# lasgroup/Model-based-policy-optimizers

Measured on AMD Instinct MI355X. Metric: model-rollout transitions/sec + SAC updates/sec, Pendulum 5-ens h=5, higher is better.
Workload: dtype f32

## Files before the change

model-based-policy-optimizers_amd/csrc/lean_blocks.hpp:

```cpp
#pragma once
#include "common.hpp"
#include "chain_run.hpp"

#define MFMA(a, b, c) __builtin_amdgcn_mfma_f32_16x16x4f32((a), (b), (c), 0, 0, 0)

constexpr int LH = 64;
constexpr int LDH = 68;
constexpr int LT = 16 * LDH;
constexpr int LDX = 8;
constexpr int HID = LH * LH + LH;

struct ImgF {
  float w[16];
  float b[4];
};
__device__ __forceinline__ void img_fwd_request(ImgF &I, const float *__restrict__ W, int c0, int lane) {
  const int i = lane & 15, g = lane >> 4;
  const float *p = W + (16 * g) * LH + c0 + i;
#pragma unroll
  for (int s = 0; s < 16; ++s) I.w[s] = p[s * LH];
  const f4u t = *reinterpret_cast<const f4u *>(W + LH * LH + c0 + 4 * g);
  I.b[0] = t[0]; I.b[1] = t[1]; I.b[2] = t[2]; I.b[3] = t[3];
}
template <int N>
// ... 79 lines not shown
    }
  }
  float zv[4];
#pragma unroll
  for (int i = 0; i < 4; ++i) zv[i] = acc[i] + I.b[i];
  const int o = j * LDH + c0 + 4 * g;
  if (STORE_Z) {
    float dv[4];
    swish_and_grad4(zv, dv);
    store_vec_lds<4>(z_out + o, dv);
  } else {
    act_apply_vec<4>(zv, MBPO_ACT_SWISH);
  }
  store_vec_lds<4>(h_out + o, zv);
}
__device__ __forceinline__ void hid_fwd_jvp(const ImgF &I, const float *xin, const float *tin, float *h_out, float *t_out, int c0, int lane) {
  const int j = lane & 15, g = lane >> 4;
  float av[16], tv_in[16];
  read_row16(av, xin, lane);
  read_row16(tv_in, tin, lane);
  f32x4 acc = {0.f, 0.f, 0.f, 0.f}, tacc = {0.f, 0.f, 0.f, 0.f};
#pragma unroll
  for (int s = 0; s < 16; ++s) {
    acc = MFMA(I.w[s], av[s], acc);
    tacc = MFMA(I.w[s], tv_in[s], tacc);
  }
  float zv[4], tv[4];
#pragma unroll
  for (int i = 0; i < 4; ++i) {
    zv[i] = acc[i] + I.b[i];
    tv[i] = tacc[i];
  }
#pragma unroll
  for (int i = 0; i < 4; ++i) {
    const float sg = fast_sigmoid(zv[i]);
    tv[i] *= sg * (1.0f + zv[i] * (1.0f - sg));
    zv[i] = zv[i] * sg;
  }
  const int o = j * LDH + c0 + 4 * g;
  store_vec_lds<4>(t_out + o, tv);
  store_vec_lds<4>(h_out + o, zv);
}
__device__ __forceinline__ f32x4 out_fwd(const float (&w)[16], const float *xin, int lane) {
  float av[16];
  read_row16(av, xin, lane);
  f32x4 acc = {0.f, 0.f, 0.f, 0.f};
#pragma unroll
  for (int s = 0; s < 16; ++s) acc = MFMA(w[s], av[s], acc);
  return acc;
}
__device__ __forceinline__ void out_fwd2(const float (&w)[16], const float *xin, const float *tin, int lane, f32x4 &y, f32x4 &ty) {
  float av[16], tv[16];
  read_row16(av, xin, lane);
  read_row16(tv, tin, lane);
  f32x4 acc = {0.f, 0.f, 0.f, 0.f}, tacc = {0.f, 0.f, 0.f, 0.f};
#pragma unroll
  for (int s = 0; s < 16; ++s) {
    acc = MFMA(w[s], av[s], acc);
    tacc = MFMA(w[s], tv[s], tacc);
  }
  y = acc;
  ty = tacc;
}
template <class ST = NoSt>
__device__ __forceinline__ void hid_dgrad(const float (&w)[16], const float *din, const float *zprev, float *d_out, int k0, int lane, ST st = ST()) {
  const int j = lane & 15, g = lane >> 4;
  float av[16];
  st(0);
  read_row16(av, din, lane);
  const int o = j * LDH + k0 + 4 * g;
  float zv[4];
  load_vec_lds<4>(zprev + o, zv);
  st(1);
  f32x4 acc = {0.f, 0.f, 0.f, 0.f};
#pragma unroll
  for (int n = 0; n < 16; ++n) acc = MFMA(w[n], av[n], acc);
  float ov[4];
  st(2);
#pragma unroll
  for (int i = 0; i < 4; ++i) ov[i] = acc[i] * zv[i];
  store_vec_lds<4>(d_out + o, ov);
  st(3);
}
template <class ST = NoSt>
__device__ __forceinline__ void hid_wgrad(const float *hin, const float *delta, float *gst, int c0, int lane, ST st = ST()) {
  const int r = lane & 15, g = lane >> 4;
  st(0);
  f32x4 acc[4], accb = {0.f, 0.f, 0.f, 0.f};
#pragma unroll
  for (int a = 0; a < 4; ++a) acc[a] = (f32x4){0.f, 0.f, 0.f, 0.f};
  float hv[4][4], dv[4];
#pragma unroll
  for (int s = 0; s < 4; ++s) {
    const int row = 4 * g + s;
    load_vec_lds<4>(hin + row * LDH + 4 * r, hv[s]);
    dv[s] = delta[row * LDH + c0 + r];
  }
  const float one0 = (r == 0) ? 1.f : 0.f;
  st(1);
#pragma unroll
  for (int s = 0; s < 4; ++s) {
#pragma unroll
    for (int a = 0; a < 4; ++a) acc[a] = MFMA(dv[s], hv[s][a], acc[a]);
    accb = MFMA(dv[s], one0, accb);
  }
  st(2);
#pragma unroll
  for (int a = 0; a < 4; ++a) {
    const float ov[4] = {acc[a][0], acc[a][1], acc[a][2], acc[a][3]};
    store_vec_lds<4>(gst + (4 * r + a) * LH + 4 * (((c0 >> 2) + g + r) & 15), ov);
  }
  if (r == 0) {
    const float ov[4] = {accb[0], accb[1], accb[2], accb[3]};
    store_vec_lds<4>(gst + LH * LH + c0 + 4 * g, ov);
  }
  st(3);
}

__device__ __forceinline__ void copy_stage_out(const float *gst, float *__restrict__ gW, int t, int n_part, int q_begin = 0, int q_end = 1040) {
  for (int q = q_begin + t; q < q_end; q += n_part) {
    float v[4];
    load_vec_lds<4>(gst + 4 * q, v);
    int dst = 4 * q;
    if (q < 1024) {
      const int k = q >> 4, cc = q & 15;
      dst = k * LH + 4 * ((cc - (k >> 2)) & 15);
    }
    store_vec_global<4>(gW + dst, v);
  }
}

template <int CTRL>
__device__ __forceinline__ float dpp_shl(float v) {
  return __int_as_float(__builtin_amdgcn_update_dpp(0, __float_as_int(v), CTRL, 0xF, 0xF, true));
}
__device__ __forceinline__ float row_sum16(float v) {
  v += dpp_shl<0x108>(v);
  v += dpp_shl<0x104>(v);
  v += dpp_shl<0x102>(v);
  v += dpp_shl<0x101>(v);
  return v;
}

template <int K, bool STORE_Z, bool TANGENT>
__device__ __forceinline__ void thin_first(const float (&tw)[K + 1], const float *x, float *h0, float *z0, float *t0, int sub, int lane) {
  float xv[4][8];
#pragma unroll
  for (int i = 0; i < 4; ++i) {
    load_vec_lds<4>(x + (4 * sub + i) * LDX, *reinterpret_cast<float(*)[4]>(&xv[i][0]));
    if (K > 4) load_vec_lds<4>(x + (4 * sub + i) * LDX + 4, *reinterpret_cast<float(*)[4]>(&xv[i][4]));
  }
  float zv[4];
#pragma unroll
  for (int i = 0; i < 4; ++i) {
    float z = tw[K];
#pragma unroll
    for (int k = 0; k < K; ++k) z = fmaf(xv[i][k], tw[k], z);
    zv[i] = z;
  }
  if (TANGENT) {
    float tv[4] = {tw[K - 1], tw[K - 1], tw[K - 1], tw[K - 1]};
    act_grad_mul_vec<4>(tv, zv, MBPO_ACT_SWISH);
#pragma unroll
    for (int i = 0; i < 4; ++i) t0[(4 * sub + i) * LDH + lane] = tv[i];
  }
  if (STORE_Z) {
    float dv[4];
    swish_and_grad4(zv, dv);
#pragma unroll
    for (int i = 0; i < 4; ++i) z0[(4 * sub + i) * LDH + lane] = dv[i];
  } else {
    act_apply_vec<4>(zv, MBPO_ACT_SWISH);
  }
#pragma unroll
  for (int i = 0; i < 4; ++i) h0[(4 * sub + i) * LDH + lane] = zv[i];
}
template <int N>
__device__ __forceinline__ void thin_dgrad_last(const float (&two)[N], const float *dY, const float (&zv)[4], float *d_out, int sub, int lane) {
  float dv[4][N], sv[4];
#pragma unroll
  for (int i = 0; i < 4; ++i)
#pragma unroll
    for (int o = 0; o < N; ++o) dv[i][o] = dY[(4 * sub + i) * 4 + o];
#pragma unroll
  for (int i = 0; i < 4; ++i) {
    float s = 0.f;
#pragma unroll
    for (int o = 0; o < N; ++o) s = fmaf(dv[i][o], two[o], s);
    sv[i] = s * zv[i];
  }
#pragma unroll
  for (int i = 0; i < 4; ++i) d_out[(4 * sub + i) * LDH + lane] = sv[i];
}
__device__ __forceinline__ void thin_z_preload(float (&zv)[4], const float *z2, int sub, int lane) {
#pragma unroll
  for (int i = 0; i < 4; ++i) zv[i] = z2[(4 * sub + i) * LDH + lane];
}
template <int N>
__device__ __forceinline__ void thin_wgrad_last(const float (&hc)[16], const float *dY, float *__restrict__ gW, int sub, int lane) {
  if (sub < N) {
    float dv[16];
#pragma unroll
    for (int r = 0; r < 16; ++r) dv[r] = dY[r * 4 + sub];
    float acc = 0.f;
#pragma unroll
    for (int r = 0; r < 16; ++r) acc = fmaf(hc[r], dv[r], acc);
    gW[lane * N + sub] = acc;
  }
  if (sub == 0 && lane < N) {
    float acc = 0.f;
#pragma unroll
    for (int r = 0; r < 16; ++r) acc += dY[r * 4 + lane];
    gW[LH * N + lane] = acc;
  }
}
__device__ __forceinline__ void thin_col_preload(float (&hc)[16], const float *h2, int lane) {
#pragma unroll
  for (int r = 0; r < 16; ++r) hc[r] = h2[r * LDH + lane];
}
template <int K>
__device__ __forceinline__ void thin_wgrad_first_(const float *x, const float *d0, float *__restrict__ gW, int w8, int lane) {
  if (w8 > K) return;
  float dv[16];
#pragma unroll
  for (int r = 0; r < 16; ++r) dv[r] = d0[r * LDH + lane];
  if (w8 < K) {
    float acc = 0.f;
#pragma unroll
    for (int r = 0; r < 16; ++r) acc = fmaf(x[r * LDX + w8], dv[r], acc);
    gW[w8 * LH + lane] = acc;
  } else {
    float acc = 0.f;
#pragma unroll
    for (int r = 0; r < 16; ++r) acc += dv[r];
    gW[K * LH + lane] = acc;
  }
}

struct Img0 {
  float w[2][2];
};

__device__ __forceinline__ void in_fwd2(const Img0 &I, const float *bias, const float *x, int kc, int K, float *h_out, int c0, int lane) {
  const int j = lane & 15, g = lane >> 4;
  float xs[2];
#pragma unroll
  for (int s = 0; s < 2; ++s) {
    const int k = g * kc + s;
    const bool ok = (s < kc) && (k < K);
    const float v = x[j * LDX + (ok ? k : 0)];
    xs[s] = ok ? v : 0.f;
  }
#pragma unroll
  for (int t = 0; t < 2; ++t) {
    f32x4 acc = {0.f, 0.f, 0.f, 0.f};
    acc = MFMA(I.w[t][0], xs[0], acc);
    acc = MFMA(I.w[t][1], xs[1], acc);
    float zv[4], bv[4];
    load_vec_lds<4>(bias + c0 + 16 * t + 4 * g, bv);
#pragma unroll
    for (int q = 0; q < 4; ++q) zv[q] = acc[q] + bv[q];
    act_apply_vec<4>(zv, MBPO_ACT_SWISH);
    store_vec_lds<4>(h_out + j * LDH + c0 + 16 * t + 4 * g, zv);
  }
}

__device__ __forceinline__ void hid_fwd2(const float (&wa)[16], const float (&wb)[16], const float *bias, const float *xin, float *h_out, int c0,
                                         int lane) {
  const int j = lane & 15, g = lane >> 4;
  float av[16];
  read_row16(av, xin, lane);
  f32x4 a = {0.f, 0.f, 0.f, 0.f}, b = {0.f, 0.f, 0.f, 0.f};
#pragma unroll
  for (int s = 0; s < 16; ++s) {
    a = MFMA(wa[s], av[s], a);
    b = MFMA(wb[s], av[s], b);
  }
  float za[4], zb[4], ba[4], bb[4];
  load_vec_lds<4>(bias + c0 + 4 * g, ba);
  load_vec_lds<4>(bias + c0 + 16 + 4 * g, bb);
#pragma unroll
  for (int q = 0; q < 4; ++q) {
    za[q] = a[q] + ba[q];
    zb[q] = b[q] + bb[q];
  }
  act_apply_vec<4>(za, MBPO_ACT_SWISH);
  act_apply_vec<4>(zb, MBPO_ACT_SWISH);
  store_vec_lds<4>(h_out + j * LDH + c0 + 4 * g, za);
  store_vec_lds<4>(h_out + j * LDH + c0 + 16 + 4 * g, zb);
}
__device__ __forceinline__ void img_w_request(float (&w)[16], const float *__restrict__ W, int c0, int lane) {
  const int i = lane & 15, g = lane >> 4;
  const float *p = W + (16 * g) * LH + c0 + i;
#pragma unroll
  for (int s = 0; s < 16; ++s) w[s] = p[s * LH];
}
```

model-based-policy-optimizers_amd/csrc/sac_lean.hip:

```cpp
#include "common.hpp"
#include "chain_run.hpp"
#include "lean_blocks.hpp"
#include "sac_shared.hpp"
#include "sac_lean.hpp"

namespace {

template <int X>
struct Net {
  static constexpr int KP = X, KQ = X + 1, D = 2 * X + 4;
  static constexpr int P_W1 = KP * LH + LH, P_OUT = P_W1 + 2 * HID, P = P_OUT + LH * 2 + 2;
  static constexpr int Q_W1 = KQ * LH + LH, Q_OUT = Q_W1 + 2 * HID, Q = Q_OUT + LH + 1;
};

constexpr int O_QIN = 0;
constexpr int O_QIN2 = 128;
constexpr int O_AUX = 256;
constexpr int O_EPS = 320;
constexpr int O_EPS2 = 336;
constexpr int O_LP = 352;
constexpr int O_A = 368, O_SIG = 384, O_RAW = 400;
constexpr int O_Q = 416;
constexpr int O_DQ = 448;
constexpr int O_QOLD = 480;
constexpr int O_DY = 496;
constexpr int O_FLAG = 560;
constexpr int O_TILES = 564;
constexpr int N_TILES = 14;
constexpr int N_AUX = 3;
constexpr int LEAN_THREADS = 64 * (8 + N_AUX);
constexpr int O_STAGE = O_TILES + N_TILES * LT;
constexpr int GST = LH * LH + LH;
constexpr size_t LEAN_LDS_BYTES = (size_t)(O_STAGE + 2 * GST) * sizeof(float);

#define LEAN_STAMP(i)                                                                   \
  if (STAMPS) {                                                                         \
    if (A.stamps && tile == 0 && tid == 0) {                                            \
      unsigned long long t_;                                                            \
      asm volatile("s_memtime %0\n\ts_waitcnt lgkmcnt(0)" : "=s"(t_)::"memory");        \
      A.stamps[(trole == 1 ? 16 : 0) + (i)] = t_;                                       \
    }                                                                                   \
  }

}

#define FINE_STAMP(w, i)                                                                \
  if (STAMPS) {                                                                         \
    if (A.stamps && tile == 0 && trole == 0 && wave == (w) && lane == 0) {              \
      unsigned long long t_;                                                            \
      asm volatile("s_memtime %0\n\ts_waitcnt lgkmcnt(0)" : "=s"(t_)::"memory");        \
      A.stamps[32 + (i)] = t_;                                                          \
    }                                                                                   \
  }

template <int X, bool STAMPS>
__global__ void __launch_bounds__(LEAN_THREADS) k_sac_lean(const SacLeanArgs A) {
  extern __shared__ __align__(16) float smem[];
  using N = Net<X>;
  constexpr int D = N::D, KP = N::KP, KQ = N::KQ;
  static_assert(X >= 1 && X + 1 <= LDX, "x + u must fit an 8-column input tile");
  const int tid_ = threadIdx.x;
  const int wave = __builtin_amdgcn_readfirstlane(tid_ >> 6);
  const int c = wave >> 2, sub = wave & 3, c0 = sub * 16;
  const int trole = blockIdx.x % 3, tile = blockIdx.x / 3;
  const float *a_params = A.params, *a_target_q = A.target_q, *a_batch = A.batch, *a_norm_mean = A.norm_mean, *a_norm_std = A.norm_std;
  float *a_slab_pi = A.slab_pi, *a_slab_q = A.slab_q;
  int B = A.B;
  asm volatile("" : "+s"(a_params), "+s"(a_target_q), "+s"(a_batch), "+s"(a_norm_mean), "+s"(a_norm_std), "+s"(a_slab_pi), "+s"(a_slab_q), "+s"(B));
  const int row0 = tile * 16;
  {
    const int tid = tid_;
    LEAN_STAMP(0);
  }
  const float invB = 1.0f / (float)B;

  float *const s_qin = smem + O_QIN, *const s_qin2 = smem + O_QIN2, *const s_aux = smem + O_AUX;
  float *const tiles = smem + O_TILES;
#define TILE(n) (tiles + (n) * LT)

  auto aux_clip_words = [&]() __attribute__((always_inline)) {
    const uint4 qw0 = *reinterpret_cast<const uint4 *>(A.opt.seq), qw1 = *reinterpret_cast<const uint4 *>(A.opt.seq + 4);
    const unsigned int seq_issued = qw0.x, seq_resolved = qw0.y;
    const bool odd = (seq_issued & 1u) == 0u;
    const float q0 = __uint_as_float(odd ? qw1.y : qw0.z), q1 = __uint_as_float(odd ? qw1.z : qw0.w), q2 = __uint_as_float(odd ? qw1.w : qw1.x);
    const float lim = (A.opt.max_norm / A.opt.grad_scale) * (A.opt.max_norm / A.opt.grad_scale) * 0.9998f;
    const bool maybe = seq_issued != seq_resolved && !(q0 < lim && q1 < lim && q2 < lim);
    if (tid_ == 512) smem[O_FLAG] = maybe ? 1.f : 0.f;
    if (blockIdx.x == 0 && tid_ == 512) {
      const float count_in = A.step_count_rw[0];
      const unsigned int slot = qw0.x & 1u;
      A.opt.slot_word[0] = slot;
      float *q = reinterpret_cast<float *>(A.opt.seq) + 2 + 3 * slot;
      q[0] = 0.f; q[1] = 0.f; q[2] = 0.f;
      A.step_count_rw[0] = count_in + 1.0f;
      if (A.p2p_epoch) {
        const unsigned int ep0_in = A.p2p_epoch[0], ep1_in = A.p2p_epoch[1];
        A.p2p_epoch[0] = ep0_in + 1u;
        A.p2p_epoch[1] = ep1_in + A.p2p_blocks;
      }
    }
  };

  auto run = [&](const bool second_pass) __attribute__((always_inline)) {
    const int tid = opaque(tid_), lane = tid & 63;
    const float *const pi_p = a_params;
    const bool has_elem = tid < 16 * D;
    const int r_t = tid / D, cc_t = tid - r_t * D;
    const bool is_obs = cc_t < X, is_obs2 = cc_t >= X + 3 && cc_t < 2 * X + 3;
    const int oc_t = is_obs ? cc_t : (is_obs2 ? cc_t - (X + 3) : 0);
    float v_t = 0.f, mu_t = 0.f, sd_t = 1.f;
    if (has_elem && (trole != 1 || is_obs)) {
      const int nvalid = (B - row0 < 16 ? B - row0 : 16) * D;
      if (tid < nvalid) v_t = a_batch[(long long)row0 * D + tid];
      if (a_norm_mean && (is_obs || is_obs2)) {
        mu_t = a_norm_mean[oc_t];
        sd_t = a_norm_std[oc_t];
      }
    }
    auto tile_to_lds = [&]() __attribute__((always_inline)) {
      if (has_elem) {
        float v = v_t;
        if (a_norm_mean && (is_obs || is_obs2)) v = (v - mu_t) / sd_t;
        int dst = -1;
        if (is_obs) dst = O_QIN + r_t * LDX + cc_t;
        else if (trole != 1) {
          if (is_obs2) dst = O_QIN2 + r_t * LDX + oc_t;
          else if (cc_t == X) dst = O_QIN + r_t * LDX + X;
          else if (cc_t == X + 1) dst = O_AUX + r_t * 4 + 0;
          else if (cc_t == X + 2) dst = O_AUX + r_t * 4 + 1;
          else dst = O_AUX + r_t * 4 + 2;
        }
        if (dst >= 0) smem[dst] = v;
      }
    };
    if (wave >= 8) {
      const int ax = wave - 8;
      const bool critic = trole != 1;
      const int kq = trole >> 1;
      const RngKey rk = rng_resolve(A.seed, A.offset, A.rng_dev);
      const bool second = lane >= 16;
      const int r = lane & 15;
      const bool draws = ax == 0 && lane < (critic ? 16 : 32);
      const float *const given = critic ? A.noise_critic : (second ? A.noise_alpha : A.noise_actor);
      const unsigned int stream = critic ? MBPO_STREAM_SAC_CRITIC : (second ? MBPO_STREAM_SAC_ALPHA : MBPO_STREAM_SAC_ACTOR);
      const long long nidx = row0 + r;
      float e_given = 0.f;
      if (draws && given && row0 + r < B) e_given = given[nidx];
      __syncthreads();
      if (ax == 0 && !second_pass) aux_clip_words();
      __syncthreads();
      Philox4 bits;
      bits.v[0] = bits.v[1] = bits.v[2] = bits.v[3] = 0u;
      if (draws && !given) bits = philox_normal_bits(rk.seed, rk.offset, stream, (unsigned long long)nidx);
      __syncthreads();
      if (draws) {
        float e = 0.f;
        if (row0 + r < B) e = given ? e_given : philox_normal_from_bits(bits);
        smem[(second ? O_EPS2 : O_EPS) + r] = e;
      }
      __syncthreads();
      __syncthreads();
      __syncthreads();
      __syncthreads();
      const float log_alpha_v = second_pass ? __hip_atomic_load(a_params + N::P + 2 * N::Q, __ATOMIC_RELAXED, __HIP_MEMORY_SCOPE_AGENT)
                                            : a_params[N::P + 2 * N::Q];
      const float alpha = expf(log_alpha_v);
      const bool ok = row0 + r < B;
      if (critic) {
        float nlp = 0.f;
        nlp += smem[O_LP + r];
        const float rew = s_aux[r * 4 + 0], disc = s_aux[r * 4 + 1], trunc = s_aux[r * 4 + 2], qold = smem[O_QOLD + r];
        float gamma = A.discounting;
        if (A.neq) {
          const float pseudo = s_qin[r * LDX + X];
          float tfa = (A.neq_tu - A.neq_tl) / 2.0f * pseudo + (A.neq_tu + A.neq_tl) / 2.0f;
          tfa = floor_divide_f(tfa, A.neq_dt) * A.neq_dt;
          gamma = expf(-A.neq_cd * tfa);
        }
        __syncthreads();
        __syncthreads();
        float e2 = 0.f;
        if (ax == 0 && lane < 16) {
          const float nq = fminf(smem[O_Q + r], smem[O_Q + 16 + r]);
          const float next_v = nq - alpha * nlp;
          const float target = rew * A.reward_scaling + disc * gamma * next_v;
          const float err = ok ? (qold - target) * (1.f - trunc) : 0.f;
          e2 = err * err;
          smem[O_DY + r * 4] = err * (1.f - trunc) * (0.5f * invB);
        }
        const float acc = row_sum16(e2);
        if (ax == 0 && lane == 0) A.slab_ex[tile * 4 + (kq == 1 ? 3 : 0)] = acc;
      } else {
        float lp_al = 0.f, lp_ac = 0.f;
        lp_al += smem[O_EPS2 + r];
        lp_ac += smem[O_LP + r];
        const float a = smem[O_A + r], sg = smem[O_SIG + r], eps = smem[O_EPS + r], raw = smem[O_RAW + r];
        __syncthreads();
        __syncthreads();
        float l_al = 0.f, l_ac = 0.f;
        if (ax == 0 && lane < 16) {
          l_al = ok ? alpha * (-lp_al - A.target_entropy) : 0.f;
          const float q0 = smem[O_Q + r], q1 = smem[O_Q + 16 + r];
          const float mq = fminf(q0, q1);
          l_ac = ok ? (alpha * lp_ac - mq) : 0.f;
          float g0 = 0.f, g1 = 0.f;
          if (ok) {
            if (q0 < q1) g0 = -invB;
            else if (q1 < q0) g1 = -invB;
            else g0 = g1 = -0.5f * invB;
          }
          const float dLda = g0 * smem[O_DQ + r] + g1 * smem[O_DQ + 16 + r];
          const float gz = dLda * (1.f - a * a) + alpha * invB * 2.f * a;
          const float gsig = gz * eps - alpha * invB / sg;
          smem[O_DY + r * 4] = ok ? gz : 0.f;
          smem[O_DY + r * 4 + 1] = ok ? gsig * fast_sigmoid(raw) : 0.f;
        }
        const float al = row_sum16(l_al), ac = row_sum16(l_ac);
        if (ax == 0 && lane == 0) {
          A.slab_ex[tile * 4 + 1] = ac;
          A.slab_ex[tile * 4 + 2] = al;
        }
      }
      __syncthreads();
      __syncthreads();
      __syncthreads();
      float *const aslab = critic ? a_slab_q + (long long)tile * (2 * N::Q) + kq * N::Q : a_slab_pi + (long long)tile * N::P;
      const int w1 = critic ? N::Q_W1 : N::P_W1, kk = critic ? KQ : KP;
      FINE_STAMP(8, 16);
      copy_stage_out(smem + O_STAGE, aslab + w1 + HID, ax * 64 + lane, N_AUX * 64);
      FINE_STAMP(8, 17);
      __syncthreads();
      FINE_STAMP(8, 18);
      copy_stage_out(smem + O_STAGE + GST, aslab + w1, (7 - kk + ax) * 64 + lane, (7 - kk + N_AUX) * 64);
      FINE_STAMP(8, 19);
    } else if (trole != 1) {
      const int kq = trole >> 1;
      const float *const qk_p = a_params + N::P + kq * N::Q;
      const float *const qt_p = a_target_q + c * N::Q;
      float tw[KQ + 1];
      ImgF I1, I2;
      float wo[16];
      float bo0 = 0.f, bo1 = 0.f;
      if (c == 0) {
        thin_col_request<KP>(*reinterpret_cast<float(*)[KP + 1]>(&tw[0]), pi_p, lane);
        img_fwd_request(I1, pi_p + N::P_W1, c0, lane);
        if (sub == 0) {
          img_out_request<2>(wo, pi_p + N::P_OUT, lane);
          bo0 = pi_p[N::P_OUT + LH * 2];
          bo1 = pi_p[N::P_OUT + LH * 2 + 1];
        }
      } else {
        thin_col_request<KQ>(tw, qk_p, lane);
        img_fwd_request(I1, qk_p + N::Q_W1, c0, lane);
        if (sub == 1) {
          img_out_request<1>(wo, qk_p + N::Q_OUT, lane);
          bo0 = qk_p[N::Q_OUT + LH];
        }
      }
      tile_to_lds();
      __syncthreads();
      LEAN_STAMP(1);
      float tw1[KQ + 1];
      ImgF J1, J2;
      if (c == 0) thin_first<KP, false, false>(*reinterpret_cast<float(*)[KP + 1]>(&tw[0]), s_qin2, TILE(0), nullptr, nullptr, sub, lane);
      else thin_first<KQ, true, false>(tw, s_qin, TILE(7), TILE(4), nullptr, sub, lane);
      thin_col_request<KQ>(tw1, qt_p, lane);
      img_fwd_request(I2, (c == 0 ? pi_p + N::P_W1 : qk_p + N::Q_W1) + HID, c0, lane);
      __syncthreads();
      LEAN_STAMP(2);
      {
        auto pf = make_pf([&](int s) __attribute__((always_inline)) { img_fwd_request_piece(J1, qt_p + N::Q_W1, c0, lane, s); });
        if (c == 0) hid_fwd<false>(I1, TILE(0), TILE(1), nullptr, c0, lane, pf);
        else hid_fwd<true>(I1, TILE(7), TILE(8), TILE(5), c0, lane, pf);
      }
      __syncthreads();
      LEAN_STAMP(3);
      {
        auto pf = make_pf([&](int s) __attribute__((always_inline)) { img_fwd_request_piece(J2, qt_p + N::Q_W1 + HID, c0, lane, s); });
        if (c == 0) hid_fwd<false>(I2, TILE(1), TILE(0), nullptr, c0, lane, pf);
        else hid_fwd<true>(I2, TILE(8), TILE(9), TILE(6), c0, lane, pf);
      }
      __syncthreads();
      LEAN_STAMP(4);
      float wo1[16];
      float bt = 0.f;
      float two[1];
      float G2[16], G1[16];
      if (c == 0 && sub == 0) {
        const f32x4 y = out_fwd(wo, TILE(0), lane);
        const float loc = y[0] + bo0, raw = y[1] + bo1;
        const int j = lane & 15;
        const ActSample sm = normal_tanh_sample(loc, raw, smem[O_EPS + j]);
        if (lane < 16) {
          s_qin2[j * LDX + X] = sm.a;
          smem[O_LP + j] = sm.lp;
        }
      } else if (c == 1 && sub == 1) {
        const f32x4 y = out_fwd(wo, TILE(9), lane);
        if (lane < 16) smem[O_QOLD + lane] = y[0] + bo0;
      }
      if (sub == c + 1) {
        img_out_request<1>(wo1, qt_p + N::Q_OUT, lane);
        bt = qt_p[N::Q_OUT + LH];
      }
      if (c == 0) {
        two[0] = qk_p[N::Q_OUT + lane];
        img_dgrad_request(G2, qk_p + N::Q_W1 + HID, c0, lane);
        img_dgrad_request(G1, qk_p + N::Q_W1, c0, lane);
      }
      __syncthreads();
      LEAN_STAMP(5);
      thin_first<KQ, false, false>(tw1, s_qin2, TILE(2 * c), nullptr, nullptr, sub, lane);
      __syncthreads();
      LEAN_STAMP(6);
      hid_fwd<false>(J1, TILE(2 * c), TILE(2 * c + 1), nullptr, c0, lane);
      __syncthreads();
      LEAN_STAMP(7);
      hid_fwd<false>(J2, TILE(2 * c + 1), TILE(2 * c), nullptr, c0, lane);
      __syncthreads();
      LEAN_STAMP(8);
      float zq[4], hc[16];
      if (sub == c + 1) {
        const f32x4 y = out_fwd(wo1, TILE(2 * c), lane);
        if (lane < 16) smem[O_Q + 16 * c + lane] = y[0] + bt;
      }
      if (c == 0) thin_z_preload(zq, TILE(6), sub, lane);
      else if (sub == 0) thin_col_preload(hc, TILE(9), lane);
      __syncthreads();
      LEAN_STAMP(9);
      __syncthreads();
      LEAN_STAMP(10);
      float *const slab = a_slab_q + (long long)tile * (2 * N::Q) + kq * N::Q;
      if (c == 0) thin_dgrad_last<1>(two, smem + O_DY, zq, TILE(0), sub, lane);
      else if (sub == 0) thin_wgrad_last<1>(hc, smem + O_DY, slab + N::Q_OUT, sub, lane);
      __syncthreads();
      LEAN_STAMP(11);
      {
        auto st0 = [&](int i) __attribute__((always_inline)) { FINE_STAMP(0, i); };
        auto st4 = [&](int i) __attribute__((always_inline)) { FINE_STAMP(4, 8 + i); };
        if (c == 0) hid_dgrad(G2, TILE(0), TILE(5), TILE(1), c0, lane, st0);
        else hid_wgrad(TILE(8), TILE(0), smem + O_STAGE, c0, lane, st4);
      }
      FINE_STAMP(0, 4);
      FINE_STAMP(4, 12);
      __syncthreads();
      FINE_STAMP(0, 5);
      FINE_STAMP(4, 13);
      LEAN_STAMP(12);
      if (c == 0) hid_dgrad(G1, TILE(1), TILE(4), TILE(2), c0, lane);
      else hid_wgrad(TILE(7), TILE(1), smem + O_STAGE + GST, c0, lane);
      FINE_STAMP(0, 20);
      FINE_STAMP(4, 21);
      __syncthreads();
      FINE_STAMP(0, 22);
      LEAN_STAMP(13);
      if (wave <= KQ) thin_wgrad_first_<KQ>(s_qin, TILE(2), slab, wave, lane);
      else copy_stage_out(smem + O_STAGE + GST, slab + N::Q_W1, (wave - (KQ + 1)) * 64 + lane, (7 - KQ + N_AUX) * 64);
      LEAN_STAMP(14);
    } else {
      const float *const q_p = a_params + N::P + c * N::Q;
      float tw[KP + 1];
      ImgF I1, I2;
      float wo[16];
      float bo0 = 0.f, bo1 = 0.f;
      float tw1[KQ + 1];
      ImgF J1, J2;
      float wo1[16];
      float bq = 0.f;
      if (c == 0) {
        thin_col_request<KP>(tw, pi_p, lane);
        img_fwd_request(I1, pi_p + N::P_W1, c0, lane);
        if (sub == 0) {
          img_out_request<2>(wo, pi_p + N::P_OUT, lane);
          bo0 = pi_p[N::P_OUT + LH * 2];
          bo1 = pi_p[N::P_OUT + LH * 2 + 1];
        }
      }
      tile_to_lds();
      __syncthreads();
      LEAN_STAMP(1);
      if (c == 0) {
        thin_first<KP, true, false>(tw, s_qin, TILE(7), TILE(4), nullptr, sub, lane);
        thin_col_request<KQ>(tw1, q_p, lane);
        img_fwd_request(I2, pi_p + N::P_W1 + HID, c0, lane);
      } else {
        thin_col_request<KQ>(tw1, q_p, lane);
        img_fwd_request(J1, q_p + N::Q_W1, c0, lane);
        img_fwd_request(J2, q_p + N::Q_W1 + HID, c0, lane);
        if (sub == 2) {
          img_out_request<1>(wo1, q_p + N::Q_OUT, lane);
          bq = q_p[N::Q_OUT + LH];
        }
      }
      __syncthreads();
      LEAN_STAMP(2);
      if (c == 0) {
        auto pf = make_pf([&](int s) __attribute__((always_inline)) { img_fwd_request_piece(J1, q_p + N::Q_W1, c0, lane, s); });
        hid_fwd<true>(I1, TILE(7), TILE(8), TILE(5), c0, lane, pf);
      }
      __syncthreads();
      LEAN_STAMP(3);
      if (c == 0) {
        auto pf = make_pf([&](int s) __attribute__((always_inline)) { img_fwd_request_piece(J2, q_p + N::Q_W1 + HID, c0, lane, s); });
        hid_fwd<true>(I2, TILE(8), TILE(9), TILE(6), c0, lane, pf);
      }
      __syncthreads();
      LEAN_STAMP(4);
      float two[2];
      float G2[16], G1[16];
      if (wave == 0) {
        const f32x4 y = out_fwd(wo, TILE(9), lane);
        const float loc = y[0] + bo0, raw = y[1] + bo1;
        const int j = lane & 15, g = lane >> 4;
        const ActSample sm = normal_tanh_sample(loc, raw, smem[(g == 1 ? O_EPS2 : O_EPS) + j]);
        if (g == 0) {
          smem[O_LP + j] = sm.lp;
          smem[O_A + j] = sm.a;
          smem[O_SIG + j] = sm.sigma;
          smem[O_RAW + j] = raw;
          s_qin[j * LDX + X] = sm.a;
        } else if (g == 1) {
          smem[O_EPS2 + j] = sm.lp;
        }
      } else if (wave == 1) {
        img_out_request<1>(wo1, q_p + N::Q_OUT, lane);
        bq = q_p[N::Q_OUT + LH];
      }
      if (c == 0) {
        two[0] = pi_p[N::P_OUT + lane * 2];
        two[1] = pi_p[N::P_OUT + lane * 2 + 1];
        img_dgrad_request(G2, pi_p + N::P_W1 + HID, c0, lane);
        img_dgrad_request(G1, pi_p + N::P_W1, c0, lane);
      }
      __syncthreads();
      LEAN_STAMP(5);
      const int tv0 = c == 0 ? 0 : 10, tt0 = c == 0 ? 2 : 12;
      thin_first<KQ, false, true>(tw1, s_qin, TILE(tv0), nullptr, TILE(tt0), sub, lane);
      __syncthreads();
      LEAN_STAMP(6);
      hid_fwd_jvp(J1, TILE(tv0), TILE(tt0), TILE(tv0 + 1), TILE(tt0 + 1), c0, lane);
      __syncthreads();
      LEAN_STAMP(7);
      hid_fwd_jvp(J2, TILE(tv0 + 1), TILE(tt0 + 1), TILE(tv0), TILE(tt0), c0, lane);
      __syncthreads();
      LEAN_STAMP(8);
      float zq[4], hc[16];
      if (sub == c + 1) {
        f32x4 y, ty;
        out_fwd2(wo1, TILE(tv0), TILE(tt0), lane, y, ty);
        if (lane < 16) {
          smem[O_Q + 16 * c + lane] = y[0] + bq;
          smem[O_DQ + 16 * c + lane] = ty[0];
        }
      }
      if (c == 0) thin_z_preload(zq, TILE(6), sub, lane);
      else if (sub < 2 && sub != 2) thin_col_preload(hc, TILE(9), lane);
      __syncthreads();
      LEAN_STAMP(9);
      __syncthreads();
      LEAN_STAMP(10);
      float *const slab = a_slab_pi + (long long)tile * N::P;
      if (c == 0) thin_dgrad_last<2>(two, smem + O_DY, zq, TILE(0), sub, lane);
      else if (sub < 2) thin_wgrad_last<2>(hc, smem + O_DY, slab + N::P_OUT, sub, lane);
      __syncthreads();
      LEAN_STAMP(11);
      if (c == 0) hid_dgrad(G2, TILE(0), TILE(5), TILE(1), c0, lane);
      else hid_wgrad(TILE(8), TILE(0), smem + O_STAGE, c0, lane);
      __syncthreads();
      LEAN_STAMP(12);
      if (c == 0) hid_dgrad(G1, TILE(1), TILE(4), TILE(2), c0, lane);
      else hid_wgrad(TILE(7), TILE(1), smem + O_STAGE + GST, c0, lane);
      __syncthreads();
      LEAN_STAMP(13);
      if (wave <= KP) thin_wgrad_first_<KP>(s_qin, TILE(2), slab, wave, lane);
      else copy_stage_out(smem + O_STAGE + GST, slab + N::P_W1, (wave - (KP + 1)) * 64 + lane, (7 - KP + N_AUX) * 64);
      LEAN_STAMP(14);
    }
  };

  run(false);
  if (smem[O_FLAG] == 0.f) return;
  float *const s_gn = smem + O_DQ;
  __syncthreads();
  sac_group_norms(A.opt, s_gn, tid_);
  __syncthreads();
  if (s_gn[0] < A.opt.max_norm && s_gn[1] < A.opt.max_norm && s_gn[2] < A.opt.max_norm) return;
  if (blockIdx.x == 0 && tid_ == 0) A.opt.seq[SAC_CTL_CLIP_EVENTS] += 1u;
  sac_clip_fixup(A.opt, s_gn, opaque(tid_), LEAN_THREADS);
  __threadfence();
  __builtin_amdgcn_s_dcache_inv();
  __syncthreads();
  run(true);
}

namespace {

template <int X>
int launch_x(const SacLeanArgs &A, int n_tiles, hipStream_t st) {
  return mbpo_with_bool(A.stamps != nullptr, [&](auto STAMP) {
    return mbpo_launch<k_sac_lean<X, STAMP.value>>(3 * n_tiles, LEAN_THREADS, LEAN_LDS_BYTES, st, "sac_lean", A);
  });
}

}

bool sac_lean_supports(int x_dim, int u_dim, const int *policy_dims, int policy_layers, int policy_act, const int *q_dims, int q_layers, int q_act) {
  if (u_dim != 1 || x_dim < 2 || x_dim > 6) return false;
  if (policy_layers != 4 || q_layers != 4 || policy_act != MBPO_ACT_SWISH || q_act != MBPO_ACT_SWISH) return false;
  for (int l = 1; l <= 3; ++l)
    if (policy_dims[l] != LH || q_dims[l] != LH) return false;
  return policy_dims[0] == x_dim && policy_dims[4] == 2 && q_dims[0] == x_dim + 1 && q_dims[4] == 1;
}

int sac_lean_launch(const SacLeanArgs &A, int x_dim, int n_tiles, void *stream) {
  hipStream_t st = (hipStream_t)stream;
  if (x_dim == 3) return launch_x<3>(A, n_tiles, st);
  if (x_dim == 4) return launch_x<4>(A, n_tiles, st);
  if (x_dim == 2) return mbpo_launch<k_sac_lean<2, false>>(3 * n_tiles, LEAN_THREADS, LEAN_LDS_BYTES, st, "sac_lean", A);
  if (x_dim == 5) return mbpo_launch<k_sac_lean<5, false>>(3 * n_tiles, LEAN_THREADS, LEAN_LDS_BYTES, st, "sac_lean", A);
  if (x_dim == 6) return mbpo_launch<k_sac_lean<6, false>>(3 * n_tiles, LEAN_THREADS, LEAN_LDS_BYTES, st, "sac_lean", A);
  mbpo_set_error("sac_lean: x_dim %d has no instantiation", x_dim);
  return MBPO_ERR_UNSUPPORTED;
}
```

Baseline: 19.41 million.

## Fuse loss and output-layer backward into hidden-layer gradient stage in SAC kernel

Every main wave now recomputes the per-row critic and actor loss gradients redundantly. The output-layer delta is folded directly into the first hidden dgrad and wgrad, and the output-layer weights are staged in LDS. This removes the O_DY round-trip through shared memory, the separate thin dgrad and wgrad passes, and several block-wide barriers. Aux waves compute the output-layer weight gradient from the loss in registers via readlane. The cost is duplicated loss arithmetic, more register pressure, and extra shuffles and LDS reads of output weights.

```diff
diff --git a/model-based-policy-optimizers_amd/csrc/lean_blocks.hpp b/model-based-policy-optimizers_amd/csrc/lean_blocks.hpp
--- a/model-based-policy-optimizers_amd/csrc/lean_blocks.hpp
+++ b/model-based-policy-optimizers_amd/csrc/lean_blocks.hpp
@@ -185,39 +185,108 @@
   store_vec_lds<4>(d_out + o, ov);
   st(3);
 }
+template <class DV, class ST = NoSt>
+__device__ __forceinline__ void hid_wgrad_from(const float *hin, DV dvf, float *gst, int c0, int lane, ST st = ST()) {
+  const int r = lane & 15, g = lane >> 4;
+  st(0);
+  f32x4 acc[4], accb = {0.f, 0.f, 0.f, 0.f};
+#pragma unroll
+  for (int a = 0; a < 4; ++a) acc[a] = (f32x4){0.f, 0.f, 0.f, 0.f};
+  float hv[4][4], dv[4];
+#pragma unroll
+  for (int s = 0; s < 4; ++s) {
+    load_vec_lds<4>(hin + (4 * g + s) * LDH + 4 * r, hv[s]);
+    dv[s] = dvf(s);
+  }
+  const float one0 = (r == 0) ? 1.f : 0.f;
+  st(1);
+#pragma unroll
+  for (int s = 0; s < 4; ++s) {
+#pragma unroll
+    for (int a = 0; a < 4; ++a) acc[a] = MFMA(dv[s], hv[s][a], acc[a]);
+    accb = MFMA(dv[s], one0, accb);
+  }
+  st(2);
+#pragma unroll
+  for (int a = 0; a < 4; ++a) {
+    const float ov[4] = {acc[a][0], acc[a][1], acc[a][2], acc[a][3]};
+    store_vec_lds<4>(gst + (4 * r + a) * LH + 4 * (((c0 >> 2) + g + r) & 15), ov);
+  }
+  if (r == 0) {
+    const float ov[4] = {accb[0], accb[1], accb[2], accb[3]};
+    store_vec_lds<4>(gst + LH * LH + c0 + 4 * g, ov);
+  }
+  st(3);
+}
 template <class ST = NoSt>
 __device__ __forceinline__ void hid_wgrad(const float *hin, const float *delta, float *gst, int c0, int lane, ST st = ST()) {
   const int r = lane & 15, g = lane >> 4;
+  hid_wgrad_from(hin, [&](int s) __attribute__((always_inline)) { return delta[(4 * g + s) * LDH + c0 + r]; }, gst, c0, lane, st);
+}
+
+template <int N>
+__device__ __forceinline__ float delta_last(const float (&dy)[N], const float (&wrow)[N], float zd) {
+  float s = 0.f;
+#pragma unroll
+  for (int o = 0; o < N; ++o) s = fmaf(dy[o], wrow[o], s);
+  return s * zd;
+}
+template <int N>
+__device__ __forceinline__ void lds_wout_rows(float (&w)[16][N], const float *wout, int lane) {
+  const float *p = wout + 16 * N * (lane >> 4);
+  float *const f = &w[0][0];
+#pragma unroll
+  for (int q = 0; q < 4 * N; ++q) load_vec_lds<4>(p + 4 * q, *reinterpret_cast<float(*)[4]>(&f[4 * q]));
+}
+template <int N>
+__device__ __forceinline__ void rows_of_group(float (&dy4)[4][N], const float (&dy)[N], int lane) {
+  const int g = lane >> 4;
+#pragma unroll
+  for (int s = 0; s < 4; ++s)
+#pragma unroll
+    for (int o = 0; o < N; ++o) dy4[s][o] = __shfl(dy[o], 4 * g + s, 64);
+}
+template <int N, class ST = NoSt>
+__device__ __forceinline__ void hid_dgrad_out(const float (&w)[16], const float (&dy)[N], const float (&wout)[16][N], float (&zd2)[16], const float *zprev,
+                                              float *d_out, int k0, int lane, ST st = ST()) {
+  const int j = lane & 15, g = lane >> 4;
   st(0);
-  f32x4 acc[4], accb = {0.f, 0.f, 0.f, 0.f};
-#pragma unroll
-  for (int a = 0; a < 4; ++a) acc[a] = (f32x4){0.f, 0.f, 0.f, 0.f};
-  float hv[4][4], dv[4];
-#pragma unroll
-  for (int s = 0; s < 4; ++s) {
-    const int row = 4 * g + s;
-    load_vec_lds<4>(hin + row * LDH + 4 * r, hv[s]);
-    dv[s] = delta[row * LDH + c0 + r];
-  }
-  const float one0 = (r == 0) ? 1.f : 0.f;
+  const int o = j * LDH + k0 + 4 * g;
+  float zv[4];
+  load_vec_lds<4>(zprev + o, zv);
+#pragma unroll
+  for (int n = 0; n < 16; ++n) zd2[n] = delta_last<N>(dy, wout[n], zd2[n]);
   st(1);
-#pragma unroll
-  for (int s = 0; s < 4; ++s) {
-#pragma unroll
-    for (int a = 0; a < 4; ++a) acc[a] = MFMA(dv[s], hv[s][a], acc[a]);
-    accb = MFMA(dv[s], one0, accb);
-  }
+  f32x4 acc = {0.f, 0.f, 0.f, 0.f};
+#pragma unroll
+  for (int n = 0; n < 16; ++n) acc = MFMA(w[n], zd2[n], acc);
+  float ov[4];
   st(2);
 #pragma unroll
-  for (int a = 0; a < 4; ++a) {
-    const float ov[4] = {acc[a][0], acc[a][1], acc[a][2], acc[a][3]};
-    store_vec_lds<4>(gst + (4 * r + a) * LH + 4 * (((c0 >> 2) + g + r) & 15), ov);
-  }
-  if (r == 0) {
-    const float ov[4] = {accb[0], accb[1], accb[2], accb[3]};
-    store_vec_lds<4>(gst + LH * LH + c0 + 4 * g, ov);
-  }
+  for (int i = 0; i < 4; ++i) ov[i] = acc[i] * zv[i];
+  store_vec_lds<4>(d_out + o, ov);
   st(3);
+}
+template <int N, class ST = NoSt>
+__device__ __forceinline__ void hid_wgrad_out(const float *hin, const float (&dy)[4][N], const float (&wcol)[N], const float (&zd)[4], float *gst, int c0,
+                                              int lane, ST st = ST()) {
+  hid_wgrad_from(hin, [&](int s) __attribute__((always_inline)) { return delta_last<N>(dy[s], wcol, zd[s]); }, gst, c0, lane, st);
+}
+template <int N>
+__device__ __forceinline__ void out_wgrad_col(const float (&hc)[16], float dy, float *__restrict__ gW, int o, int lane) {
+  float dv[16];
+#pragma unroll
+  for (int r = 0; r < 16; ++r) dv[r] = __int_as_float(__builtin_amdgcn_readlane(__float_as_int(dy), r));
+  float acc = 0.f;
+#pragma unroll
+  for (int r = 0; r < 16; ++r) acc = fmaf(hc[r], dv[r], acc);
+  gW[lane * N + o] = acc;
+  if (lane == 0) {
+    float b = 0.f;
+#pragma unroll
+    for (int r = 0; r < 16; ++r) b += dv[r];
+    gW[LH * N + o] = b;
+  }
 }
 
 __device__ __forceinline__ void copy_stage_out(const float *gst, float *__restrict__ gW, int t, int n_part, int q_begin = 0, int q_end = 1040) {
@@ -299,24 +368,6 @@
 #pragma unroll
   for (int i = 0; i < 4; ++i) zv[i] = z2[(4 * sub + i) * LDH + lane];
 }
-template <int N>
-__device__ __forceinline__ void thin_wgrad_last(const float (&hc)[16], const float *dY, float *__restrict__ gW, int sub, int lane) {
-  if (sub < N) {
-    float dv[16];
-#pragma unroll
-    for (int r = 0; r < 16; ++r) dv[r] = dY[r * 4 + sub];
-    float acc = 0.f;
-#pragma unroll
-    for (int r = 0; r < 16; ++r) acc = fmaf(hc[r], dv[r], acc);
-    gW[lane * N + sub] = acc;
-  }
-  if (sub == 0 && lane < N) {
-    float acc = 0.f;
-#pragma unroll
-    for (int r = 0; r < 16; ++r) acc += dY[r * 4 + lane];
-    gW[LH * N + lane] = acc;
-  }
-}
 __device__ __forceinline__ void thin_col_preload(float (&hc)[16], const float *h2, int lane) {
 #pragma unroll
   for (int r = 0; r < 16; ++r) hc[r] = h2[r * LDH + lane];
diff --git a/model-based-policy-optimizers_amd/csrc/sac_lean.hip b/model-based-policy-optimizers_amd/csrc/sac_lean.hip
--- a/model-based-policy-optimizers_amd/csrc/sac_lean.hip
+++ b/model-based-policy-optimizers_amd/csrc/sac_lean.hip
@@ -23,9 +23,9 @@
 constexpr int O_Q = 416;
 constexpr int O_DQ = 448;
 constexpr int O_QOLD = 480;
-constexpr int O_DY = 496;
 constexpr int O_FLAG = 560;
-constexpr int O_TILES = 564;
+constexpr int O_WOUT = 564;
+constexpr int O_TILES = O_WOUT + 128;
 constexpr int N_TILES = 14;
 constexpr int N_AUX = 3;
 constexpr int LEAN_THREADS = 64 * (8 + N_AUX);
@@ -41,6 +41,78 @@
       A.stamps[(trole == 1 ? 16 : 0) + (i)] = t_;                                       \
     }                                                                                   \
   }
+
+struct LossArgs {
+  int neq;
+  float discounting, reward_scaling, target_entropy, neq_cd, neq_tl, neq_tu, neq_dt;
+};
+struct CriticRow {
+  float nlp, rew, disc, trunc, qold, gamma;
+};
+struct CriticLoss {
+  float dy, e2;
+};
+template <int X>
+__device__ __forceinline__ CriticRow critic_row_preload(const float *smem, const LossArgs &A, int r) {
+  CriticRow p;
+  float nlp = 0.f;
+  nlp += smem[O_LP + r];
+  p.nlp = nlp;
+  p.rew = smem[O_AUX + r * 4 + 0], p.disc = smem[O_AUX + r * 4 + 1], p.trunc = smem[O_AUX + r * 4 + 2], p.qold = smem[O_QOLD + r];
+  float gamma = A.discounting;
+  if (A.neq) {
+    const float pseudo = smem[O_QIN + r * LDX + X];
+    float tfa = (A.neq_tu - A.neq_tl) / 2.0f * pseudo + (A.neq_tu + A.neq_tl) / 2.0f;
+    tfa = floor_divide_f(tfa, A.neq_dt) * A.neq_dt;
+    gamma = expf(-A.neq_cd * tfa);
+  }
+  p.gamma = gamma;
+  return p;
+}
+__device__ __forceinline__ CriticLoss critic_loss_row(const float *smem, const CriticRow &p, float alpha, float reward_scaling, bool ok, float invB, int r) {
+  const float nq = fminf(smem[O_Q + r], smem[O_Q + 16 + r]);
+  const float next_v = nq - alpha * p.nlp;
+  const float target = p.rew * reward_scaling + p.disc * p.gamma * next_v;
+  const float err = ok ? (p.qold - target) * (1.f - p.trunc) : 0.f;
+  CriticLoss l;
+  l.e2 = err * err;
+  l.dy = err * (1.f - p.trunc) * (0.5f * invB);
+  return l;
+}
+struct ActorRow {
+  float lp_al, lp_ac, a, sg, eps, raw;
+};
+struct ActorLoss {
+  float dy[2], l_al, l_ac;
+};
+__device__ __forceinline__ ActorRow actor_row_preload(const float *smem, int r) {
+  ActorRow p;
+  float lp_al = 0.f, lp_ac = 0.f;
+  lp_al += smem[O_EPS2 + r];
+  lp_ac += smem[O_LP + r];
+  p.lp_al = lp_al, p.lp_ac = lp_ac;
+  p.a = smem[O_A + r], p.sg = smem[O_SIG + r], p.eps = smem[O_EPS + r], p.raw = smem[O_RAW + r];
+  return p;
+}
+__device__ __forceinline__ ActorLoss actor_loss_row(const float *smem, const ActorRow &p, float alpha, float target_entropy, bool ok, float invB, int r) {
+  ActorLoss l;
+  l.l_al = ok ? alpha * (-p.lp_al - target_entropy) : 0.f;
+  const float q0 = smem[O_Q + r], q1 = smem[O_Q + 16 + r];
+  const float mq = fminf(q0, q1);
+  l.l_ac = ok ? (alpha * p.lp_ac - mq) : 0.f;
+  float g0 = 0.f, g1 = 0.f;
+  if (ok) {
+    if (q0 < q1) g0 = -invB;
+    else if (q1 < q0) g1 = -invB;
+    else g0 = g1 = -0.5f * invB;
+  }
+  const float dLda = g0 * smem[O_DQ + r] + g1 * smem[O_DQ + 16 + r];
+  const float gz = dLda * (1.f - p.a * p.a) + alpha * invB * 2.f * p.a;
+  const float gsig = gz * p.eps - alpha * invB / p.sg;
+  l.dy[0] = ok ? gz : 0.f;
+  l.dy[1] = ok ? gsig * fast_sigmoid(p.raw) : 0.f;
+  return l;
+}
 
 }
 
@@ -67,6 +139,9 @@
   float *a_slab_pi = A.slab_pi, *a_slab_q = A.slab_q;
   int B = A.B;
   asm volatile("" : "+s"(a_params), "+s"(a_target_q), "+s"(a_batch), "+s"(a_norm_mean), "+s"(a_norm_std), "+s"(a_slab_pi), "+s"(a_slab_q), "+s"(B));
+  LossArgs LA = {A.neq, A.discounting, A.reward_scaling, A.target_entropy, A.neq_cd, A.neq_tl, A.neq_tu, A.neq_dt};
+  asm volatile("" : "+s"(LA.neq), "+s"(LA.discounting), "+s"(LA.reward_scaling), "+s"(LA.target_entropy), "+s"(LA.neq_cd), "+s"(LA.neq_tl), "+s"(LA.neq_tu),
+               "+s"(LA.neq_dt));
   const int row0 = tile * 16;
   {
     const int tid = tid_;
@@ -74,7 +149,7 @@
   }
   const float invB = 1.0f / (float)B;
 
-  float *const s_qin = smem + O_QIN, *const s_qin2 = smem + O_QIN2, *const s_aux = smem + O_AUX;
+  float *const s_qin = smem + O_QIN, *const s_qin2 = smem + O_QIN2;
   float *const tiles = smem + O_TILES;
 #define TILE(n) (tiles + (n) * LT)
 
@@ -133,6 +208,9 @@
         if (dst >= 0) smem[dst] = v;
       }
     };
+    auto load_log_alpha = [&]() __attribute__((always_inline)) {
+      return second_pass ? __hip_atomic_load(a_params + N::P + 2 * N::Q, __ATOMIC_RELAXED, __HIP_MEMORY_SCOPE_AGENT) : a_params[N::P + 2 * N::Q];
+    };
     if (wave >= 8) {
       const int ax = wave - 8;
       const bool critic = trole != 1;
@@ -148,6 +226,12 @@
       if (draws && given && row0 + r < B) e_given = given[nidx];
       __syncthreads();
       if (ax == 0 && !second_pass) aux_clip_words();
+      const float *const wout_p = critic ? a_params + N::P + kq * N::Q + N::Q_OUT : a_params + N::P_OUT;
+      float wout0 = 0.f, wout1 = 0.f;
+      if (ax == 1) {
+        wout0 = wout_p[lane];
+        if (!critic) wout1 = wout_p[64 + lane];
+      }
       __syncthreads();
       Philox4 bits;
       bits.v[0] = bits.v[1] = bits.v[2] = bits.v[3] = 0u;
@@ -158,73 +242,46 @@
         if (row0 + r < B) e = given ? e_given : philox_normal_from_bits(bits);
         smem[(second ? O_EPS2 : O_EPS) + r] = e;
       }
-      __syncthreads();
-      __syncthreads();
-      __syncthreads();
-      __syncthreads();
-      const float log_alpha_v = second_pass ? __hip_atomic_load(a_params + N::P + 2 * N::Q, __ATOMIC_RELAXED, __HIP_MEMORY_SCOPE_AGENT)
-                                            : a_params[N::P + 2 * N::Q];
-      const float alpha = expf(log_alpha_v);
+      if (ax == 1) {
+        smem[O_WOUT + lane] = wout0;
+        if (!critic) smem[O_WOUT + 64 + lane] = wout1;
+      }
+      __syncthreads();
+      __syncthreads();
+      __syncthreads();
+      __syncthreads();
+      const float alpha = expf(load_log_alpha());
       const bool ok = row0 + r < B;
+      float *const aslab = critic ? a_slab_q + (long long)tile * (2 * N::Q) + kq * N::Q : a_slab_pi + (long long)tile * N::P;
+      float hc[16];
+      if (ax >= 1) thin_col_preload(hc, TILE(9), lane);
       if (critic) {
-        float nlp = 0.f;
-        nlp += smem[O_LP + r];
-        const float rew = s_aux[r * 4 + 0], disc = s_aux[r * 4 + 1], trunc = s_aux[r * 4 + 2], qold = smem[O_QOLD + r];
-        float gamma = A.discounting;
-        if (A.neq) {
-          const float pseudo = s_qin[r * LDX + X];
-          float tfa = (A.neq_tu - A.neq_tl) / 2.0f * pseudo + (A.neq_tu + A.neq_tl) / 2.0f;
-          tfa = floor_divide_f(tfa, A.neq_dt) * A.neq_dt;
-          gamma = expf(-A.neq_cd * tfa);
-        }
+        const CriticRow pr = critic_row_preload<X>(smem, LA, r);
         __syncthreads();
         __syncthreads();
-        float e2 = 0.f;
-        if (ax == 0 && lane < 16) {
-          const float nq = fminf(smem[O_Q + r], smem[O_Q + 16 + r]);
-          const float next_v = nq - alpha * nlp;
-          const float target = rew * A.reward_scaling + disc * gamma * next_v;
-          const float err = ok ? (qold - target) * (1.f - trunc) : 0.f;
-          e2 = err * err;
-          smem[O_DY + r * 4] = err * (1.f - trunc) * (0.5f * invB);
-        }
-        const float acc = row_sum16(e2);
-        if (ax == 0 && lane == 0) A.slab_ex[tile * 4 + (kq == 1 ? 3 : 0)] = acc;
+        const CriticLoss l = critic_loss_row(smem, pr, alpha, LA.reward_scaling, ok, invB, r);
+        if (ax == 0) {
+          const float acc = row_sum16(lane < 16 ? l.e2 : 0.f);
+          if (lane == 0) A.slab_ex[tile * 4 + (kq == 1 ? 3 : 0)] = acc;
+        } else if (ax == 1) {
+          out_wgrad_col<1>(hc, l.dy, aslab + N::Q_OUT, 0, lane);
+        }
       } else {
-        float lp_al = 0.f, lp_ac = 0.f;
-        lp_al += smem[O_EPS2 + r];
-        lp_ac += smem[O_LP + r];
-        const float a = smem[O_A + r], sg = smem[O_SIG + r], eps = smem[O_EPS + r], raw = smem[O_RAW + r];
+        const ActorRow pr = actor_row_preload(smem, r);
         __syncthreads();
         __syncthreads();
-        float l_al = 0.f, l_ac = 0.f;
-        if (ax == 0 && lane < 16) {
-          l_al = ok ? alpha * (-lp_al - A.target_entropy) : 0.f;
-          const float q0 = smem[O_Q + r], q1 = smem[O_Q + 16 + r];
-          const float mq = fminf(q0, q1);
-          l_ac = ok ? (alpha * lp_ac - mq) : 0.f;
-          float g0 = 0.f, g1 = 0.f;
-          if (ok) {
-            if (q0 < q1) g0 = -invB;
-            else if (q1 < q0) g1 = -invB;
-            else g0 = g1 = -0.5f * invB;
+        const ActorLoss l = actor_loss_row(smem, pr, alpha, LA.target_entropy, ok, invB, r);
+        if (ax == 0) {
+          const float al = row_sum16(lane < 16 ? l.l_al : 0.f), ac = row_sum16(lane < 16 ? l.l_ac : 0.f);
+          if (lane == 0) {
+            A.slab_ex[tile * 4 + 1] = ac;
+            A.slab_ex[tile * 4 + 2] = al;
           }
-          const float dLda = g0 * smem[O_DQ + r] + g1 * smem[O_DQ + 16 + r];
-          const float gz = dLda * (1.f - a * a) + alpha * invB * 2.f * a;
-          const float gsig = gz * eps - alpha * invB / sg;
-          smem[O_DY + r * 4] = ok ? gz : 0.f;
-          smem[O_DY + r * 4 + 1] = ok ? gsig * fast_sigmoid(raw) : 0.f;
-        }
-        const float al = row_sum16(l_al), ac = row_sum16(l_ac);
-        if (ax == 0 && lane == 0) {
-          A.slab_ex[tile * 4 + 1] = ac;
-          A.slab_ex[tile * 4 + 2] = al;
-        }
-      }
-      __syncthreads();
-      __syncthreads();
-      __syncthreads();
-      float *const aslab = critic ? a_slab_q + (long long)tile * (2 * N::Q) + kq * N::Q : a_slab_pi + (long long)tile * N::P;
+        } else {
+          out_wgrad_col<2>(hc, ax == 1 ? l.dy[0] : l.dy[1], aslab + N::P_OUT, ax - 1, lane);
+        }
+      }
+      __syncthreads();
       const int w1 = critic ? N::Q_W1 : N::P_W1, kk = critic ? KQ : KP;
       FINE_STAMP(8, 16);
       copy_stage_out(smem + O_STAGE, aslab + w1 + HID, ax * 64 + lane, N_AUX * 64);
@@ -284,7 +341,6 @@
       LEAN_STAMP(4);
       float wo1[16];
       float bt = 0.f;
-      float two[1];
       float G2[16], G1[16];
       if (c == 0 && sub == 0) {
         const f32x4 y = out_fwd(wo, TILE(0), lane);
@@ -304,10 +360,10 @@
         bt = qt_p[N::Q_OUT + LH];
       }
       if (c == 0) {
-        two[0] = qk_p[N::Q_OUT + lane];
         img_dgrad_request(G2, qk_p + N::Q_W1 + HID, c0, lane);
         img_dgrad_request(G1, qk_p + N::Q_W1, c0, lane);
       }
+      const float log_alpha_v = load_log_alpha();
       __syncthreads();
       LEAN_STAMP(5);
       thin_first<KQ, false, false>(tw1, s_qin2, TILE(2 * c), nullptr, nullptr, sub, lane);
@@ -319,44 +375,53 @@
       hid_fwd<false>(J2, TILE(2 * c + 1), TILE(2 * c), nullptr, c0, lane);
       __syncthreads();
       LEAN_STAMP(8);
-      float zq[4], hc[16];
+      const int lj = lane & 15, lg = lane >> 4;
       if (sub == c + 1) {
         const f32x4 y = out_fwd(wo1, TILE(2 * c), lane);
         if (lane < 16) smem[O_Q + 16 * c + lane] = y[0] + bt;
       }
-      if (c == 0) thin_z_preload(zq, TILE(6), sub, lane);
-      else if (sub == 0) thin_col_preload(hc, TILE(9), lane);
+      const float alpha = expf(log_alpha_v);
+      const CriticRow pr = critic_row_preload<X>(smem, LA, lj);
+      float wrow[16][1], wcol[1], zd2[16], zdw[4];
+      if (c == 0) {
+        read_row16(zd2, TILE(6), lane);
+        lds_wout_rows<1>(wrow, smem + O_WOUT, lane);
+      } else {
+        wcol[0] = smem[O_WOUT + c0 + lj];
+#pragma unroll
+        for (int s = 0; s < 4; ++s) zdw[s] = TILE(6)[(4 * lg + s) * LDH + c0 + lj];
+      }
       __syncthreads();
       LEAN_STAMP(9);
-      __syncthreads();
-      LEAN_STAMP(10);
       float *const slab = a_slab_q + (long long)tile * (2 * N::Q) + kq * N::Q;
-      if (c == 0) thin_dgrad_last<1>(two, smem + O_DY, zq, TILE(0), sub, lane);
-      else if (sub == 0) thin_wgrad_last<1>(hc, smem + O_DY, slab + N::Q_OUT, sub, lane);
-      __syncthreads();
-      LEAN_STAMP(11);
       {
         auto st0 = [&](int i) __attribute__((always_inline)) { FINE_STAMP(0, i); };
         auto st4 = [&](int i) __attribute__((always_inline)) { FINE_STAMP(4, 8 + i); };
-        if (c == 0) hid_dgrad(G2, TILE(0), TILE(5), TILE(1), c0, lane, st0);
-        else hid_wgrad(TILE(8), TILE(0), smem + O_STAGE, c0, lane, st4);
+        const float dy[1] = {critic_loss_row(smem, pr, alpha, LA.reward_scaling, row0 + lj < B, invB, lj).dy};
+        if (c == 0) {
+          hid_dgrad_out<1>(G2, dy, wrow, zd2, TILE(5), TILE(1), c0, lane, st0);
+        } else {
+          float dy4[4][1];
+          rows_of_group<1>(dy4, dy, lane);
+          hid_wgrad_out<1>(TILE(8), dy4, wcol, zdw, smem + O_STAGE, c0, lane, st4);
+        }
       }
       FINE_STAMP(0, 4);
       FINE_STAMP(4, 12);
       __syncthreads();
       FINE_STAMP(0, 5);
       FINE_STAMP(4, 13);
-      LEAN_STAMP(12);
+      LEAN_STAMP(10);
       if (c == 0) hid_dgrad(G1, TILE(1), TILE(4), TILE(2), c0, lane);
       else hid_wgrad(TILE(7), TILE(1), smem + O_STAGE + GST, c0, lane);
       FINE_STAMP(0, 20);
       FINE_STAMP(4, 21);
       __syncthreads();
       FINE_STAMP(0, 22);
-      LEAN_STAMP(13);
+      LEAN_STAMP(11);
       if (wave <= KQ) thin_wgrad_first_<KQ>(s_qin, TILE(2), slab, wave, lane);
       else copy_stage_out(smem + O_STAGE + GST, slab + N::Q_W1, (wave - (KQ + 1)) * 64 + lane, (7 - KQ + N_AUX) * 64);
-      LEAN_STAMP(14);
+      LEAN_STAMP(12);
     } else {
       const float *const q_p = a_params + N::P + c * N::Q;
       float tw[KP + 1];
@@ -406,7 +471,6 @@
       }
       __syncthreads();
       LEAN_STAMP(4);
-      float two[2];
       float G2[16], G1[16];
       if (wave == 0) {
         const f32x4 y = out_fwd(wo, TILE(9), lane);
@@ -427,11 +491,10 @@
         bq = q_p[N::Q_OUT + LH];
       }
       if (c == 0) {
-        two[0] = pi_p[N::P_OUT + lane * 2];
-        two[1] = pi_p[N::P_OUT + lane * 2 + 1];
         img_dgrad_request(G2, pi_p + N::P_W1 + HID, c0, lane);
         img_dgrad_request(G1, pi_p + N::P_W1, c0, lane);
       }
+      const float log_alpha_v = load_log_alpha();
       __syncthreads();
       LEAN_STAMP(5);
       const int tv0 = c == 0 ? 0 : 10, tt0 = c == 0 ? 2 : 12;
@@ -444,7 +507,7 @@
       hid_fwd_jvp(J2, TILE(tv0 + 1), TILE(tt0 + 1), TILE(tv0), TILE(tt0), c0, lane);
       __syncthreads();
       LEAN_STAMP(8);
-      float zq[4], hc[16];
+      const int lj = lane & 15, lg = lane >> 4;
       if (sub == c + 1) {
         f32x4 y, ty;
         out_fwd2(wo1, TILE(tv0), TILE(tt0), lane, y, ty);
@@ -453,28 +516,40 @@
           smem[O_DQ + 16 * c + lane] = ty[0];
         }
       }
-      if (c == 0) thin_z_preload(zq, TILE(6), sub, lane);
-      else if (sub < 2 && sub != 2) thin_col_preload(hc, TILE(9), lane);
+      const float alpha = expf(log_alpha_v);
+      const ActorRow pr = actor_row_preload(smem, lj);
+      float wrow[16][2], wcol[2], zd2[16], zdw[4];
+      if (c == 0) {
+        read_row16(zd2, TILE(6), lane);
+        lds_wout_rows<2>(wrow, smem + O_WOUT, lane);
+      } else {
+        wcol[0] = smem[O_WOUT + (c0 + lj) * 2];
+        wcol[1] = smem[O_WOUT + (c0 + lj) * 2 + 1];
+#pragma unroll
+        for (int s = 0; s < 4; ++s) zdw[s] = TILE(6)[(4 * lg + s) * LDH + c0 + lj];
+      }
       __syncthreads();
       LEAN_STAMP(9);
+      float *const slab = a_slab_pi + (long long)tile * N::P;
+      {
+        const ActorLoss l = actor_loss_row(smem, pr, alpha, LA.target_entropy, row0 + lj < B, invB, lj);
+        if (c == 0) {
+          hid_dgrad_out<2>(G2, l.dy, wrow, zd2, TILE(5), TILE(1), c0, lane);
+        } else {
+          float dy4[4][2];
+          rows_of_group<2>(dy4, l.dy, lane);
+          hid_wgrad_out<2>(TILE(8), dy4, wcol, zdw, smem + O_STAGE, c0, lane);
+        }
+      }
       __syncthreads();
       LEAN_STAMP(10);
-      float *const slab = a_slab_pi + (long long)tile * N::P;
-      if (c == 0) thin_dgrad_last<2>(two, smem + O_DY, zq, TILE(0), sub, lane);
-      else if (sub < 2) thin_wgrad_last<2>(hc, smem + O_DY, slab + N::P_OUT, sub, lane);
-      __syncthreads();
-      LEAN_STAMP(11);
-      if (c == 0) hid_dgrad(G2, TILE(0), TILE(5), TILE(1), c0, lane);
-      else hid_wgrad(TILE(8), TILE(0), smem + O_STAGE, c0, lane);
-      __syncthreads();
-      LEAN_STAMP(12);
       if (c == 0) hid_dgrad(G1, TILE(1), TILE(4), TILE(2), c0, lane);
       else hid_wgrad(TILE(7), TILE(1), smem + O_STAGE + GST, c0, lane);
       __syncthreads();
-      LEAN_STAMP(13);
+      LEAN_STAMP(11);
       if (wave <= KP) thin_wgrad_first_<KP>(s_qin, TILE(2), slab, wave, lane);
       else copy_stage_out(smem + O_STAGE + GST, slab + N::P_W1, (wave - (KP + 1)) * 64 + lane, (7 - KP + N_AUX) * 64);
-      LEAN_STAMP(14);
+      LEAN_STAMP(12);
     }
   };
 
```

New measurement: 19.61 million (median of 6 runs). 1.01x the previous value.
